# patrickltobing/shallow-wavenet

Measured on AMD Instinct MI355X. Metric: decoded samples/sec (22.05 kHz Laplacian AR decode, whole job), higher is better.
Workload: dtype f32

## Files before the change

shallow_wavenet_amd/csrc/swn_decode_bl6w.hip:

```cpp
#include <type_traits>
#include "swn_decode_bl6_common.hpp"
#include "swn_decode_internal.hpp"

namespace {

using namespace swn_bl6;

constexpr int NG = 256;
constexpr int S = 128;
constexpr int O1 = 128;

template <int LPC_, bool EXT_>
struct Tw {
    static constexpr int LPC = LPC_;
    static constexpr bool EXT = EXT_;
    using Ext = Tw<LPC_, true>;
    static constexpr int NO = 2 + LPC_;
    static constexpr int WN = cmax(1, LPC_) + 1;
    static constexpr int ring_len(int l) { return pow2ceil((1 << l) + 1); }
    static constexpr int ring_off(int l) { int o = 0; for (int i = 0; i < l; ++i) o += ring_len(i) * H; return o; }
    static constexpr int PF = L * 2 * H;
    static constexpr int NZC = 64, NZB = 4;
    static constexpr int o_ring = 0;
    static constexpr int o_hcat = o_ring + ring_off(L);
    static constexpr int o_gp = o_hcat + L * H;
    static constexpr int o_bx = o_gp + 2 * PF;
    static constexpr int o_bd = o_bx + L * 2 * H;
    static constexpr int o_old = o_bd + L * 2 * H;
    static constexpr int o_wup = o_old + 2 * L * 2 * H;
    static constexpr int o_skip = o_wup + 256;
    static constexpr int o_p2 = o_skip + S;
    static constexpr int o_tnz = o_p2 + 4 * NO;
    static constexpr int o_cz = o_tnz + r4(NZB * NZC);
    static constexpr int o_w2 = o_cz + 5 * H;
    static constexpr int o_bias = o_w2 + NO * S + r4(NO);
    static constexpr int o_w1 = o_bias + S + O1;
    static constexpr int o_wl = o_w1 + 8 * O1 * 16;
    static constexpr int o_h0w = o_wl + 8 * NG * 4;
    static constexpr int o_end = o_h0w + 3 * H;
    static constexpr size_t lds_bytes = (size_t)o_end * sizeof(float);
    static constexpr int sess_old = ring_off(L);
    static constexpr int sess_win = sess_old + 2 * L * 2 * H;
    static constexpr int sess_floats = sess_win + r4(WN);
};

__device__ __forceinline__ float sum_quads(float v) {
    v += dpp_f<0x124>(v);
    v += dpp_f<0x128>(v);
    float w = v;
    asm("s_nop 1\n\tv_permlane16_swap_b32 %0, %1" : "+v"(v), "+v"(w));
    v += w;
    w = v;
    asm("s_nop 1\n\tv_permlane32_swap_b32 %0, %1" : "+v"(v), "+v"(w));
    return v + w;
}
template <class T, int LAYER>
__device__ __forceinline__ void layer_a(float* lds, const float (&w)[2][16], const int q, const float wj, const int pb, const int ta,
                                        const float* xr) {
    const int o = ta >> 2, p = ta & 3, pr = p & 1;
    const float e_old = lds[T::o_old + (q & 1) * (L * 2 * H) + LAYER * 2 * H + pr * H + o];
    const float e_gx = fmaf(wj, lds[T::o_gp + pb + LAYER * 2 * H + pr * H + o], lds[T::o_bx + LAYER * 2 * H + pr * H + o]);
    const float e_hp = xr[o];
    float az = 0.f, ac = 0.f;
#pragma unroll
    for (int m = 0; m < 4; ++m) {
        const float4 x = *reinterpret_cast<const float4*>(xr + 16 * p + 4 * m);
        az = fmaf(w[0][4 * m], x.x, az); ac = fmaf(w[1][4 * m], x.x, ac);
        az = fmaf(w[0][4 * m + 1], x.y, az); ac = fmaf(w[1][4 * m + 1], x.y, ac);
        az = fmaf(w[0][4 * m + 2], x.z, az); ac = fmaf(w[1][4 * m + 2], x.z, ac);
        az = fmaf(w[0][4 * m + 3], x.w, az); ac = fmaf(w[1][4 * m + 3], x.w, ac);
    }
    az = sum4(az); ac = sum4(ac);
    __builtin_amdgcn_sched_barrier(0);
    if (p < 2) {
        const float sa = (p == 0 ? az : ac) + e_old;
        const float v = e_gx * sa;
        float res;
        if (fabsf(v) > 9.02f && p == 1) {
            res = copysignf(1.f, v);
        } else {
            const float e = exp_c(p == 0 ? -v : -2.f * fabsf(v));
            const float r = rcp_c(1.f + e);
            res = p == 0 ? r : copysignf((1.f - e) * r, v);
        }
        const float c = dpp_f<0xF5>(res);
        if (p == 0) {
            const float hn = (1.f - res) * c + res * e_hp;
            if (LAYER + 1 < L) {
                constexpr int R2 = T::ring_len(LAYER + 1 < L ? LAYER + 1 : LAYER);
                lds[T::o_ring + T::ring_off(LAYER + 1 < L ? LAYER + 1 : LAYER) + (q & (R2 - 1)) * H + o] = hn;
            }
            lds[T::o_hcat + LAYER * H + o] = hn;
        }
    }
    __builtin_amdgcn_sched_barrier(0);
}

template <class T, int LAYER, int MB = 4>
__device__ __forceinline__ void older_sum(const float* lds, const float (&w)[2][16], const int qn, const int tb, float& az, float& ac) {
    constexpr int dil = 1 << LAYER;
    constexpr int R = T::ring_len(LAYER);
    const int p = tb & 3;
    const float* ring = lds + T::o_ring + T::ring_off(LAYER);
    az = 0.f; ac = 0.f;
#pragma unroll
    for (int m = 0; m < 4; ++m) {
        const float4 x = *reinterpret_cast<const float4*>(ring + ((qn - dil) & (R - 1)) * H + 16 * p + 4 * m);
        float4 w0, w1;
        if (LAYER < L - 1) {
            w0 = make_float4(w[0][4 * m], w[0][4 * m + 1], w[0][4 * m + 2], w[0][4 * m + 3]);
            w1 = make_float4(w[1][4 * m], w[1][4 * m + 1], w[1][4 * m + 2], w[1][4 * m + 3]);
        } else {
            w0 = *reinterpret_cast<const float4*>(lds + T::o_wl + (m * NG + tb) * 4);
            w1 = *reinterpret_cast<const float4*>(lds + T::o_wl + ((4 + m) * NG + tb) * 4);
        }
        az = fmaf(w0.x, x.x, az); ac = fmaf(w1.x, x.x, ac);
        az = fmaf(w0.y, x.y, az); ac = fmaf(w1.y, x.y, ac);
        az = fmaf(w0.z, x.z, az); ac = fmaf(w1.z, x.z, ac);
        az = fmaf(w0.w, x.w, az); ac = fmaf(w1.w, x.w, ac);
        if (MB < 4 && m % MB == MB - 1) __builtin_amdgcn_sched_barrier(0);
    }
    az = sum4(az); ac = sum4(ac);
}
template <class T, int LAYER>
__device__ __forceinline__ void older_store(float* lds, const int qn, const int tb, const float az, const float ac) {
    const int o = tb >> 2, p = tb & 3, pr = p & 1;
    lds[T::o_old + (qn & 1) * (L * 2 * H) + LAYER * 2 * H + pr * H + o] = (p == 0 ? az : ac) + lds[T::o_bd + LAYER * 2 * H + pr * H + o];
}
template <class T, int LAYER, int MB = 4>
__device__ __forceinline__ void older_b(float* lds, const float (&w)[2][16], const int qn, const int tb) {
    float az, ac;
    older_sum<T, LAYER, MB>(lds, w, qn, tb, az, ac);
    if ((tb & 3) < 2) older_store<T, LAYER>(lds, qn, tb, az, ac);
}
template <int... LS> struct Layers {};
template <class T, int NW, int... LS>
__device__ __forceinline__ void older_bn(Layers<LS...>, float* lds, const float (&w)[NW][2][16], const int qn, const int tb) {
    static_assert(((LS < NW) && ...), "register-resident halves only");
    float az[sizeof...(LS)], ac[sizeof...(LS)];
    int k = 0;
    ((older_sum<T, LS>(lds, w[LS], qn, tb, az[k], ac[k]), ++k), ...);
    if ((tb & 3) < 2) {
        k = 0;
        ((older_store<T, LS>(lds, qn, tb, az[k], ac[k]), ++k), ...);
    }
}

template <class T, int LAYER>
__device__ __forceinline__ void older_rows(const float* lds, const int qn, const int tb, float4 (&x)[4]) {
    constexpr int dil = 1 << LAYER;
    constexpr int R = T::ring_len(LAYER);
    const float* row = lds + T::o_ring + T::ring_off(LAYER) + ((qn - dil) & (R - 1)) * H + 16 * (tb & 3);
#pragma unroll
    for (int m = 0; m < 4; ++m) x[m] = *reinterpret_cast<const float4*>(row + 4 * m);
}
__device__ __forceinline__ void older_sum_x(const float (&w)[2][16], const float4 (&x)[4], float& az, float& ac) {
    az = 0.f; ac = 0.f;
#pragma unroll
    for (int m = 0; m < 4; ++m) {
        az = fmaf(w[0][4 * m], x[m].x, az); ac = fmaf(w[1][4 * m], x[m].x, ac);
        az = fmaf(w[0][4 * m + 1], x[m].y, az); ac = fmaf(w[1][4 * m + 1], x[m].y, ac);
        az = fmaf(w[0][4 * m + 2], x[m].z, az); ac = fmaf(w[1][4 * m + 2], x[m].z, ac);
        az = fmaf(w[0][4 * m + 3], x[m].w, az); ac = fmaf(w[1][4 * m + 3], x[m].w, ac);
    }
    az = sum4(az); ac = sum4(ac);
}
template <class T, int... LS>
__device__ __forceinline__ void older_rows_n(Layers<LS...>, const float* lds, const int qn, const int tb, float4 (&x)[sizeof...(LS)][4]) {
    int k = 0;
    ((older_rows<T, LS>(lds, qn, tb, x[k]), ++k), ...);
}
template <class T, int NW, int... LS>
__device__ __forceinline__ void older_bn_x(Layers<LS...>, float* lds, const float (&w)[NW][2][16], const float4 (&x)[sizeof...(LS)][4],
                                           const int qn, const int tb) {
    static_assert(((LS < NW) && ...), "register-resident halves only");
    float az[sizeof...(LS)], ac[sizeof...(LS)];
    int k = 0;
    ((older_sum_x(w[LS], x[k], az[k], ac[k]), ++k), ...);
    if ((tb & 3) < 2) {
        k = 0;
        ((older_store<T, LS>(lds, qn, tb, az[k], ac[k]), ++k), ...);
    }
}

template <int LAYER>
__device__ __forceinline__ void skip_issue_b(__amdgpu_buffer_rsrc_t wsk2, float4 (&wsl)[8], const int tb, const unsigned step0) {
    const int r = tb >> 2, hp = tb & 3;
#pragma unroll
    for (int ps = 0; ps < 2; ++ps)
#pragma unroll
        for (int mm = 0; mm < 4; ++mm)
            wsl[ps * 4 + mm] = buf_ld4(wsk2, (unsigned)((r + 64 * ps) * 4 + hp) * 16u, (unsigned)((LAYER * 4 + mm) * S) * 64u + step0);
}
template <class T, int LAYER>
__device__ __forceinline__ void skip_roll_b(const float* lds, __amdgpu_buffer_rsrc_t wsk2, float4 (&wsl)[8], float (&sacc)[2], const int tb,
                                            const unsigned step0) {
    static_assert(LAYER >= 1 && LAYER < L, "slice LAYER - 1 in flight, slice LAYER to request");
    const int r = tb >> 2, hp = tb & 3;
#pragma unroll
    for (int hf = 0; hf < 2; ++hf) {
#pragma unroll
        for (int mm = 2 * hf; mm < 2 * hf + 2; ++mm) {
            const float4 x = *reinterpret_cast<const float4*>(lds + T::o_hcat + (LAYER - 1) * H + 16 * mm + 4 * hp);
#pragma unroll
            for (int ps = 0; ps < 2; ++ps) {
                const float4 w = wsl[ps * 4 + mm];
                sacc[ps] = fmaf(w.x, x.x, sacc[ps]); sacc[ps] = fmaf(w.y, x.y, sacc[ps]);
                sacc[ps] = fmaf(w.z, x.z, sacc[ps]); sacc[ps] = fmaf(w.w, x.w, sacc[ps]);
            }
        }
        __builtin_amdgcn_sched_barrier(0);
#pragma unroll
        for (int mm = 2 * hf; mm < 2 * hf + 2; ++mm)
#pragma unroll
            for (int ps = 0; ps < 2; ++ps)
                wsl[ps * 4 + mm] = buf_ld4(wsk2, (unsigned)((r + 64 * ps) * 4 + hp) * 16u, (unsigned)((LAYER * 4 + mm) * S) * 64u + step0);
        __builtin_amdgcn_sched_barrier(0);
    }
    asm volatile("" : "+v"(sacc[0]), "+v"(sacc[1]));
}
template <class T>
__device__ __forceinline__ void skip_last_b(float* lds, const float4 (&wsl)[8], const float (&sacc)[2], const int tb) {
    const int r = tb >> 2, hp = tb & 3;
    float part[2][4];
#pragma unroll
    for (int mm = 0; mm < 4; ++mm) {
        const float4 x = *reinterpret_cast<const float4*>(lds + T::o_hcat + (L - 1) * H + 16 * mm + 4 * hp);
#pragma unroll
        for (int ps = 0; ps < 2; ++ps) {
            const float4 w = wsl[ps * 4 + mm];
            part[ps][mm] = fmaf(w.w, x.w, fmaf(w.z, x.z, fmaf(w.y, x.y, w.x * x.x)));
        }
    }
    float s[2];
#pragma unroll
    for (int ps = 0; ps < 2; ++ps) s[ps] = sacc[ps] + ((part[ps][0] + part[ps][1]) + (part[ps][2] + part[ps][3]));
    const float t0 = s[0] + dpp_f<0xB1>(s[0]), t1 = s[1] + dpp_f<0xB1>(s[1]);
    const float v = (hp < 2 ? t0 : t1) + dpp_f<0x4E>(hp < 2 ? t1 : t0);
    if ((hp & 1) == 0) lds[T::o_skip + r + 32 * hp] = fmaxf(v, 0.f);
}

using OlderMerged = Layers<3, 4>;
using OlderOut1 = Layers<0, 1, 2>;

template <class T, bool GA, bool STREAM, bool POOL = false>
__device__ __forceinline__ void decode_body(const Bl6Args& a, float* lds) {
    constexpr bool EXT = T::EXT;
    static_assert(!STREAM || EXT, "streamed chunks run the extended mode");
    constexpr bool grpA = GA;
    const int tid = threadIdx.x, b = POOL ? 0 : blockIdx.x;
    __builtin_assume(GA ? tid < NG : tid >= NG);
    const int tg = tid & (NG - 1);
    const float* __restrict__ P = a.P;
    const int U = a.U;
    const int s0 = STREAM ? a.step0 : 0;
    const bool resume = STREAM && a.resume;
    const int fb0 = STREAM ? s0 / U : 0;

    for (int e = tid; e < T::o_end; e += NT) lds[e] = 0.f;
    __syncthreads();
    for (int e = tid; e < L * 2 * H; e += NT) {
        lds[T::o_bx + e] = P[a.y.bx + e];
        const float bd = P[a.y.bd + e];
        lds[T::o_bd + e] = bd;
        lds[T::o_old + e] = bd;
    }
    for (int e = tid; e < U; e += NT) lds[T::o_wup + e] = P[a.y.wup + e];
    for (int e = tid; e < H; e += NT) lds[T::o_cz + e] = P[a.y.cb + e];
    for (int e = tid; e < S; e += NT) lds[T::o_bias + e] = P[a.y.bsk + e];
    for (int e = tid; e < O1; e += NT) lds[T::o_bias + S + e] = P[a.y.b1 + e];
    for (int e = tid; e < 2 * H; e += NT) { lds[T::o_cz + H + e] = P[a.y.cv + e]; lds[T::o_cz + 3 * H + e] = P[a.y.cc + e]; }
    for (int e = tid; e < T::NO * S; e += NT) lds[T::o_w2 + e] = P[a.y.w2 + (size_t)(e / S) * r4(S) + (e % S)];
    for (int e = tid; e < T::NO; e += NT) lds[T::o_w2 + T::NO * S + e] = P[a.y.b2 + e];
    for (int e = tid; e < 8 * O1 * 16; e += NT) lds[T::o_w1 + e] = P[a.y.w12 + e];
    const __amdgpu_buffer_rsrc_t condr =
        make_rsrc(a.cond + (size_t)b * a.Tf * a.N, (unsigned)((size_t)a.Tf * a.N * sizeof(float)));
    auto load_frame = [&](int fr) {
        float* dst = lds + T::o_gp + (fr & 1) * T::PF;
#pragma unroll
        for (int it = 0; it < (T::PF / 4 + NT - 1) / NT; ++it) {
            const int e4 = it * NT + tid;
            if (e4 < T::PF / 4)
                *reinterpret_cast<float4*>(dst + 4 * e4) =
                    buf_ld4(condr, (unsigned)tid * 16u, (unsigned)(fr * a.N * 4 + it * NT * 16));
        }
    };
    for (int fr = fb0; fr < fb0 + 2 && fr < a.Tf; ++fr) load_frame(fr);
    constexpr int NWR = grpA ? L : L - 1;
    float wreg[NWR][2][16];
    {
        const int o = tg >> 2, p = tg & 3, k = grpA ? 1 : 0;
#pragma unroll
        for (int l = 0; l < L; ++l)
#pragma unroll
            for (int r = 0; r < 2; ++r) {
                const float4* src = reinterpret_cast<const float4*>(P + a.y.wd + (((size_t)l * 2 * H + o + r * H) * 2 + k) * H + 16 * p);
#pragma unroll
                for (int v = 0; v < 4; ++v) {
                    const float4 t = src[v];
                    if (l == L - 1 && !grpA) {
                        *reinterpret_cast<float4*>(lds + T::o_wl + ((r * 4 + v) * NG + tg) * 4) = t;
                    } else {
                        float (&wr)[16] = wreg[l < NWR ? l : 0][r];
                        wr[4 * v] = t.x; wr[4 * v + 1] = t.y; wr[4 * v + 2] = t.z; wr[4 * v + 3] = t.w;
                    }
                }
            }
    }
    __syncthreads();
    const float* sess_b = STREAM ? a.sess + (size_t)b * T::sess_floats : nullptr;
    int tcp = tid;
    asm volatile("" : "+v"(tcp));
    if (resume) {
        for (int e = tcp; e < T::ring_off(L); e += NT) lds[T::o_ring + e] = sess_b[e];
        for (int e = tcp; e < 2 * L * 2 * H; e += NT) lds[T::o_old + e] = sess_b[T::sess_old + e];
        __syncthreads();
    }

    int fb = fb0, tb0 = fb0 * U;
    const int n_pro = RF;
    auto cond_taps = [&](int q, float& wj, int& pb) {
        const int t0 = q - RF;
        const int tlo = t0 < 0 ? 0 : t0;
        if (tlo >= tb0 + U) {
            fb += 1; tb0 += U;
            if (fb + 1 < a.Tf) load_frame(fb + 1);
        }
        int rel = tlo - tb0;
        int fsel = fb;
        if (rel >= U) { rel -= U; fsel = fb + 1; }
        rel = rel < U ? rel : U - 1;
        wj = lds[T::o_wup + rel];
        pb = (fsel & 1) * T::PF;
    };

    auto input_seed = [&](int q) {
        if (tid < H) {
            const int o = tid;
            float acc = c_b;
#pragma unroll
            for (int k = 0; k < 2; ++k) {
                const int r = q - (1 - k);
                if (r >= 0) acc += fmaf(k ? c_v1 : c_v0, 0.f, k ? c_c1 : c_c0);
            }
            lds[T::o_ring + (q & 1) * H + o] = ssign(acc);
        }
    };
    float win[T::WN];
#pragma unroll
    for (int k = 0; k < T::WN; ++k) win[k] = 0.f;
    if (EXT && a.seed) win[T::WN - 1] = reinterpret_cast<const float*>(a.seed)[b];
    if (resume) {
#pragma unroll
        for (int k = 0; k < T::WN; ++k) win[k] = sess_b[T::sess_win + k];
    }
    const int wv = __builtin_amdgcn_readfirstlane(tg >> 6);
    float kcb = 0.f, kv0 = 0.f, kv1 = 0.f, kc0 = 0.f, kc1 = 0.f;
    if (grpA) { const int o = tg & (H - 1); kcb = c_b; kv0 = c_v0; kv1 = c_v1; kc0 = c_c0; kc1 = c_c1; }
    auto h0_row = [&](int qn) -> float* {
        return wv == 0 ? lds + T::o_ring + (qn & 1) * H : lds + T::o_h0w + (wv - 1) * H;
    };
    auto input_gen = [&](int qn) {
        if constexpr (grpA) {
            float acc = kcb;
            acc += fmaf(kv0, win[T::WN - 2], kc0);
            acc += fmaf(kv1, win[T::WN - 1], kc1);
            h0_row(qn)[tg & (H - 1)] = ssign(acc);
            asm volatile("s_waitcnt lgkmcnt(0)" ::: "memory");
        }
    };
    float e_next = 0.f;
    auto noise_load = [&](int c) {
        const int step = c * T::NZC + tid - 64;
        if (step < a.n_steps) e_next = a.noise[(size_t)b * a.n_steps + step];
    };
    auto noise_chunk = [&](int c) {
        if (grpA && tid >= 64 && tid < 128) {
            const int k = tid - 64, step = c * T::NZC + k;
            if (step < a.n_steps) {
                const float e = EXT ? swn_noise_laplace_at(a.nz, b, step, s0 + step, 0, a.n_steps, 1) : e_next;
                const float sg = (e > 0.f) ? 1.f : ((e < 0.f) ? -1.f : 0.f);
                lds[T::o_tnz + (c & (T::NZB - 1)) * T::NZC + k] = sg * log1pf(-2.f * fabsf(e));
            }
            if (!EXT) noise_load(c + 1);
        }
    };
    if (!EXT && grpA && tid >= 64 && tid < 128) noise_load(0);
    noise_chunk(0);
    noise_chunk(1);

    const __amdgpu_buffer_rsrc_t wsk2 = make_rsrc(P + a.y.wsk2, (unsigned)(L * S * 64 * sizeof(float)));

#ifdef SWN_STAMP
    unsigned long long tw[9] = {0, 0, 0, 0, 0, 0, 0, 0, 0}, tv[6] = {0, 0, 0, 0, 0, 0}, tstep = 0, tlast = 0, tbeg = 0;
#define SWN_BAR(k) { tw[k] += __builtin_amdgcn_s_memtime() - tlast; lds_barrier(); tlast = __builtin_amdgcn_s_memtime(); }
#define SWN_WAIT_STAMP(k) { asm volatile("" :: "v"(wsl[0].x)); tv[k] += __builtin_amdgcn_s_memtime() - tlast; }
#define SWN_PRE(k) { tw[k] += __builtin_amdgcn_s_memtime() - tlast; asm volatile("s_waitcnt lgkmcnt(0)" ::: "memory"); }
#define SWN_BAR_KEEP(k, N) { lds_barrier_keep<N>(); tlast = __builtin_amdgcn_s_memtime(); }
#else
#define SWN_BAR(k) lds_barrier();
#define SWN_WAIT_STAMP(k)
#define SWN_PRE(k)
#define SWN_BAR_KEEP(k, N) lds_barrier_keep<N>();
#endif
#define SWN_PHASE(LAYER, GEN, X0)                                                                                     \
    if constexpr (grpA) layer_a<T, LAYER>(lds, wreg[LAYER], q, wj, pb, tg,                                             \
                                          LAYER == 0 ? (X0) : lds + T::o_ring + T::ring_off(LAYER) +                   \
                                                                  (q & (T::ring_len(LAYER) - 1)) * H);                 \
    else {                                                                                                             \
        if (GEN) {    \
                      \
                      \
            if (LAYER == 0) skip_issue_b<0>(wsk2, wsl, tg, step0);                                                     \
            else { SWN_WAIT_STAMP(LAYER > 0 ? LAYER - 1 : 0) skip_roll_b<T, (LAYER > 0 ? LAYER : 1)>(lds, wsk2, wsl, sacc, tg, step0); } \
            __builtin_amdgcn_sched_barrier(0);                                                                         \
        }                                                                                                              \
        if (!(GEN)) older_b<T, LAYER>(lds, wreg[LAYER < NWR ? LAYER : 0], q + 1, tg);                                  \
        else if (LAYER == 0) older_bn<T>(OlderMerged{}, lds, wreg, q + 1, tg);                                         \
        __builtin_amdgcn_sched_barrier(0);                                                                             \
    }                                                                                                                  \
    if (GEN) { SWN_BAR(LAYER) } else lds_barrier();

#pragma unroll 1
    for (int q = resume ? n_pro : 0; q < n_pro; ++q) {
        float wj; int pb;
        float4 wsl[8]; float sacc[2]; const unsigned step0 = 0;
        cond_taps(q, wj, pb);
        input_seed(q);
        lds_barrier();
        const float* x0 = lds + T::o_ring + (q & 1) * H;
        SWN_PHASE(0, false, x0) SWN_PHASE(1, false, x0) SWN_PHASE(2, false, x0) SWN_PHASE(3, false, x0)
        SWN_PHASE(4, false, x0) SWN_PHASE(5, false, x0)
        (void)wsl; (void)sacc; (void)step0;
    }

    input_gen(RF + s0);
#ifdef SWN_STAMP
    tlast = tbeg = __builtin_amdgcn_s_memtime();
#endif
    auto gen_step = [&](const int i) __attribute__((always_inline)) {
        const int q = RF + s0 + i;
        float wj; int pb;
        cond_taps(q, wj, pb);
        float4 wsl[8];
        float sacc[2] = {0.f, 0.f};
        if constexpr (!grpA) {
            const float bs0 = lds[T::o_bias + (tg >> 2)], bs1 = lds[T::o_bias + (tg >> 2) + 64];
            if ((tg & 3) == 0) { sacc[0] = bs0; sacc[1] = bs1; }
        }
        unsigned step0 = 0;
        asm volatile("" : "+s"(step0));
        const float* x0 = h0_row(q);
        SWN_PHASE(0, true, x0) SWN_PHASE(1, true, x0) SWN_PHASE(2, true, x0) SWN_PHASE(3, true, x0)
        SWN_PHASE(4, true, x0) SWN_PHASE(5, true, x0)
        constexpr bool ROLL1 = T::LPC == 0;
        float4 xo[3][4];
        float4 w1e[2][2];
        if constexpr (!grpA) {
            SWN_WAIT_STAMP(5) skip_last_b<T>(lds, wsl, sacc, tg);
            SWN_PRE(6)
            lds_fence_compiler();
            __builtin_amdgcn_sched_barrier(0);
            older_rows_n<T>(OlderOut1{}, lds, q + 1, tg, xo);
            __builtin_amdgcn_sched_barrier(0);
            SWN_BAR_KEEP(6, 12)
        } else {
            older_b<T, L - 1, 2>(lds, wreg[L - 1], q + 1, tg + (int)step0);
            if constexpr (ROLL1) {
                SWN_PRE(6)
                lds_fence_compiler();
                __builtin_amdgcn_sched_barrier(0);
#pragma unroll
                for (int mm = 0; mm < 2; ++mm)
#pragma unroll
                    for (int r = 0; r < 2; ++r)
                        w1e[mm][r] = *reinterpret_cast<const float4*>(lds + T::o_w1 + ((mm * O1 + (tg >> 2) + 64 * r) * 4 + (tg & 3)) * 4);
                __builtin_amdgcn_sched_barrier(0);
                SWN_BAR_KEEP(6, 4)
            } else {
                SWN_BAR(6)
            }
        }
        if constexpr (grpA) {
            const int hr = tg >> 2, hp = tg & 3;
            float a0 = 0.f, a1 = 0.f, b0 = 0.f, b1 = 0.f;
            auto X = [&](int mm) { return *reinterpret_cast<const float4*>(lds + T::o_skip + 16 * mm + 4 * hp); };
            auto W = [&](int mm, int r) { return *reinterpret_cast<const float4*>(lds + T::o_w1 + ((mm * O1 + hr + 64 * r) * 4 + hp) * 4); };
            auto fma8 = [&](int mm, const float4& x0, const float4& w0, const float4& w1) {
                float& acc = (mm & 1) ? a1 : a0;
                float& bcc = (mm & 1) ? b1 : b0;
                acc = fmaf(w0.x, x0.x, acc); acc = fmaf(w0.y, x0.y, acc); acc = fmaf(w0.z, x0.z, acc); acc = fmaf(w0.w, x0.w, acc);
                bcc = fmaf(w1.x, x0.x, bcc); bcc = fmaf(w1.y, x0.y, bcc); bcc = fmaf(w1.z, x0.z, bcc); bcc = fmaf(w1.w, x0.w, bcc);
            };
            if constexpr (ROLL1) {
                float4 xr[3] = {X(0), X(1), X(2)};
                __builtin_amdgcn_sched_barrier(0);
#pragma unroll
                for (int mm = 0; mm < 8; ++mm) {
                    fma8(mm, xr[mm % 3], w1e[mm % 2][0], w1e[mm % 2][1]);
                    __builtin_amdgcn_sched_barrier(0);
                    if (mm + 2 < 8) { w1e[mm % 2][0] = W(mm + 2, 0); w1e[mm % 2][1] = W(mm + 2, 1); }
                    if (mm + 3 < 8) xr[mm % 3] = X(mm + 3);
                    __builtin_amdgcn_sched_barrier(0);
                }
            } else {
#pragma unroll
                for (int mm = 0; mm < 8; ++mm) {
                    fma8(mm, X(mm), W(mm, 0), W(mm, 1));
                    if ((mm & 3) == 3) __builtin_amdgcn_sched_barrier(0);
                }
            }
            const float v = sum4(a0 + a1), u = sum4(b0 + b1);
            const float o1a = fmaxf(v + lds[T::o_bias + S + hr], 0.f), o1b = fmaxf(u + lds[T::o_bias + S + hr + 64], 0.f);
#pragma unroll
            for (int j = 0; j < (T::NO + 3) / 4; ++j) {
                const int k = hp + 4 * j, kc = k < T::NO ? k : T::NO - 1;
                const float* w2 = lds + T::o_w2 + kc * S;
                const float b2 = lds[T::o_w2 + T::NO * S + kc];
                const float pz = sum_quads(fmaf(w2[hr + 64], o1b, fmaf(w2[hr], o1a, tg < 4 ? b2 : 0.f)));
                if ((tg & 63) < 4 && k < T::NO) lds[T::o_p2 + 4 * k + wv] = pz;
            }
        } else {
            older_bn_x<T>(OlderOut1{}, lds, wreg, xo, q + 1, tg);
        }
        SWN_BAR(7)
        if constexpr (grpA) {
            const int ln = tg & 63;
            float tz = 0.f;
            if constexpr (!EXT) tz = lds[T::o_tnz + (i & (T::NZB * T::NZC - 1))];
            float fv = 0.f;
            if (a.forced) fv = reinterpret_cast<const float*>(a.forced)[(size_t)b * a.n_steps + i];
            const float4 pz = *reinterpret_cast<const float4*>(lds + T::o_p2 + 4 * (ln < T::NO ? ln : T::NO - 1));
            const float acc = (pz.x + pz.y) + (pz.z + pz.w);
            float o2[T::NO];
#pragma unroll
            for (int k = 0; k < T::NO; ++k) o2[k] = __builtin_bit_cast(float, __builtin_amdgcn_readlane(__builtin_bit_cast(int, acc), k));
            {
#pragma clang fp contract(off)
                float* outp = reinterpret_cast<float*>(a.out) + (size_t)b * a.n_steps + (size_t)i;
                const float mu = o2[0];
                const float bsc = sigm(o2[1]);
                float lpv = 0.f;
#pragma unroll
                for (int k = 0; k < T::LPC; ++k) lpv += o2[2 + T::LPC - 1 - k] * win[T::WN - T::LPC + k];
                const float t = bsc * (EXT ? lds[T::o_tnz + ((i >> 6) & (T::NZB - 1)) * T::NZC + (i & (T::NZC - 1))] : tz);
                float sv = (T::LPC > 0) ? (lpv + mu) - t : mu - t;
                sv = fminf(fmaxf(sv, -1.f), 1.f);
                float fd = a.forced ? fv : sv;
                asm volatile("" : "+v"(fd));
#pragma unroll
                for (int k = 0; k + 1 < T::WN; ++k) win[k] = win[k + 1];
                win[T::WN - 1] = fd;
                if (tid == 0) outp[0] = sv;
            }
            if (HEADS_ON && a.heads && wv == 0 && ln < T::NO) a.heads[((size_t)b * a.n_steps + i) * T::NO + ln] = acc;
        }
        if (i + 1 < a.n_steps) input_gen(q + 1);
#ifdef SWN_STAMP
        if constexpr (grpA) tw[8] += __builtin_amdgcn_s_memtime() - tlast;
#endif
    };
#pragma unroll 1
    for (int i0 = 0; i0 < a.n_steps; i0 += T::NZC) {
        noise_chunk((i0 >> 6) + 2);
        const int iend = i0 + T::NZC < a.n_steps ? i0 + T::NZC : a.n_steps;
#pragma unroll 1
        for (int i = i0; i < iend; ++i) gen_step(i);
    }
#ifdef SWN_STAMP
    { const unsigned long long tn = __builtin_amdgcn_s_memtime(); tw[0] += tn - tlast; tstep = tn - tbeg; }
#endif
    if constexpr (STREAM) {
        __syncthreads();
        float* so = a.sess + (size_t)b * T::sess_floats;
        tcp = tid;
        asm volatile("" : "+v"(tcp));
        for (int e = tcp; e < T::ring_off(L); e += NT) so[e] = lds[T::o_ring + e];
        for (int e = tcp; e < 2 * L * 2 * H; e += NT) so[T::sess_old + e] = lds[T::o_old + e];
        if (tid == 0) {
#pragma unroll
            for (int k = 0; k < T::WN; ++k) so[T::sess_win + k] = win[k];
        }
    }
#undef SWN_PHASE
#undef SWN_BAR
#undef SWN_WAIT_STAMP
#undef SWN_PRE
#undef SWN_BAR_KEEP
#ifdef SWN_STAMP
    if ((tid == 0 || tid == 64 || tid == NG) && b == 0 && a.heads) {
        float* h = a.heads + (tid == 0 ? 0 : tid == 64 ? 30 : 10);
        for (int k = 0; k < 9; ++k) h[k] = (float)((double)tw[k] / (double)a.n_steps);
        if (tid == 0) h[9] = (float)((double)tstep / (double)a.n_steps);
        else if (tid == NG) for (int k = 0; k < 6; ++k) h[10 + k] = (float)((double)tv[k] / (double)a.n_steps);
    }
#endif
}

template <class T, bool STREAM = false>
__global__ __launch_bounds__(NT) void decode_bl6w_kernel(const Bl6Args a) {
    extern __shared__ __attribute__((aligned(16))) float lds[];
    if (threadIdx.x < NG) decode_body<T, true, STREAM>(a, lds);
    else decode_body<T, false, STREAM>(a, lds);
}

template <class T, bool MODELS = false>
__global__ __launch_bounds__(NT) void decode_bl6w_pool_kernel(
    const typename std::conditional<MODELS, Bl6PoolModelsArgs, Bl6PoolArgs>::type p) {
    extern __shared__ __attribute__((aligned(16))) float lds[];
    static_assert(T::EXT, "pools run the extended mode");
    Bl6Args a = p.c;
    if constexpr (MODELS) a.P = swn_pool_model(p.m);
    if (!swn_pool_entry_args(a, p.t, 1, 1, T::NO)) return;
    a.sess += (size_t)swn_pool_slot(p.t) * T::sess_floats;
    if (threadIdx.x < NG) decode_body<T, true, true, true>(a, lds);
    else decode_body<T, false, true, true>(a, lds);
}

bool bl6w_applies(const SwnGeom& g) {
    return g.bl6 && g.U <= 256 && g.U >= 2 && !g.audio_in && g.kind == SWN_KIND_LAPLACE && g.S == 128 && g.O1 == 128 &&
           g.seg == 1 && (g.lpc == 0 || g.lpc == 4);
}

template <class F>
int with_tw(const SwnGeom& g, F&& f) {
    if (!bl6w_applies(g)) return SWN_E_UNSUPPORTED;
    if (g.lpc == 0) return f(Tw<0, false>{});
    return f(Tw<4, false>{});
}

}

int swn_decode_bl6w_run(const SwnDecodeCall& c) {
    const hipStream_t st = c.hip_stream;
    if (c.pool) {
        Bl6PoolModelsArgs p;
        fill_args(p.c, c);
        p.t = *c.pool;
        if (c.models) p.m = *c.models;
        return with_tw(c.g, [&](auto tw) {
            using T = typename decltype(tw)::Ext;
            if (c.models)
                return launch_kernel(decode_bl6w_pool_kernel<T, true>, T::lds_bytes, c.batch, p, st, "swn_decode_pool_chunk_models(bl6w)");
            const Bl6PoolArgs& p1 = p;
            return launch_kernel(decode_bl6w_pool_kernel<T>, T::lds_bytes, c.batch, p1, st, "swn_decode_pool_chunk(bl6w)");
        });
    }
    Bl6Args a;
    fill_args(a, c);
    return with_tw(c.g, [&](auto t) {
        using T = decltype(t);
        using X = typename T::Ext;
        static_assert(T::lds_bytes <= 160 * 1024 && X::lds_bytes <= 160 * 1024, "LDS budget");
        if (c.stream) return launch_kernel(decode_bl6w_kernel<X, true>, X::lds_bytes, a.B, a, st, "swn_decode(bl6w)");
        if (wants_ext(a)) return launch_kernel(decode_bl6w_kernel<X>, X::lds_bytes, a.B, a, st, "swn_decode(bl6w)");
        return launch_kernel(decode_bl6w_kernel<T>, T::lds_bytes, a.B, a, st, "swn_decode(bl6w)");
    });
}

size_t swn_decode_bl6w_session_floats(const SwnGeom& g) {
    int n = 0;
    with_tw(g, [&](auto t) { n = decltype(t)::sess_floats; return SWN_OK; });
    return (size_t)n;
}
```

Before: 373,800.

## Precompute next-step conditioning taps and prefetch out_2 weights in decode loop

```diff
diff --git a/shallow_wavenet_amd/csrc/swn_decode_bl6w.hip b/shallow_wavenet_amd/csrc/swn_decode_bl6w.hip
--- a/shallow_wavenet_amd/csrc/swn_decode_bl6w.hip
+++ b/shallow_wavenet_amd/csrc/swn_decode_bl6w.hip
@@ -55,10 +55,10 @@
     return v + w;
 }
 template <class T, int LAYER>
-__device__ __forceinline__ void layer_a(float* lds, const float (&w)[2][16], const int q, const float wj, const int pb, const int ta,
-                                        const float* xr) {
+__device__ __forceinline__ void layer_a(float* lds, const float (&w)[2][16], const int q, const float wj, const int pb, const int po,
+                                        const int ta, const float* xr) {
     const int o = ta >> 2, p = ta & 3, pr = p & 1;
-    const float e_old = lds[T::o_old + (q & 1) * (L * 2 * H) + LAYER * 2 * H + pr * H + o];
+    const float e_old = lds[T::o_old + po + LAYER * 2 * H + pr * H + o];
     const float e_gx = fmaf(wj, lds[T::o_gp + pb + LAYER * 2 * H + pr * H + o], lds[T::o_bx + LAYER * 2 * H + pr * H + o]);
     const float e_hp = xr[o];
     float az = 0.f, ac = 0.f;
@@ -357,16 +357,16 @@
     const int wv = __builtin_amdgcn_readfirstlane(tg >> 6);
     float kcb = 0.f, kv0 = 0.f, kv1 = 0.f, kc0 = 0.f, kc1 = 0.f;
     if (grpA) { const int o = tg & (H - 1); kcb = c_b; kv0 = c_v0; kv1 = c_v1; kc0 = c_c0; kc1 = c_c1; }
-    auto h0_row = [&](int qn) -> float* {
-        return wv == 0 ? lds + T::o_ring + (qn & 1) * H : lds + T::o_h0w + (wv - 1) * H;
-    };
-    auto input_gen = [&](int qn) {
+    auto h0_row = [&](int qn) -> int {
+        return wv == 0 ? T::o_ring + (qn & 1) * H : T::o_h0w + (wv - 1) * H;
+    };
+    auto input_gen = [&](int row) {
         if constexpr (grpA) {
             float acc = kcb;
             acc += fmaf(kv0, win[T::WN - 2], kc0);
             acc += fmaf(kv1, win[T::WN - 1], kc1);
-            h0_row(qn)[tg & (H - 1)] = ssign(acc);
-            asm volatile("s_waitcnt lgkmcnt(0)" ::: "memory");
+            lds[row + (tg & (H - 1))] = ssign(acc);
+            lds_fence_compiler();
         }
     };
     float e_next = 0.f;
@@ -404,7 +404,7 @@
 #define SWN_BAR_KEEP(k, N) lds_barrier_keep<N>();
 #endif
 #define SWN_PHASE(LAYER, GEN, X0)                                                                                     \
-    if constexpr (grpA) layer_a<T, LAYER>(lds, wreg[LAYER], q, wj, pb, tg,                                             \
+    if constexpr (grpA) layer_a<T, LAYER>(lds, wreg[LAYER], q, wj, pb, po, tg,                                         \
                                           LAYER == 0 ? (X0) : lds + T::o_ring + T::ring_off(LAYER) +                   \
                                                                   (q & (T::ring_len(LAYER) - 1)) * H);                 \
     else {                                                                                                             \
@@ -426,6 +426,7 @@
         float wj; int pb;
         float4 wsl[8]; float sacc[2]; const unsigned step0 = 0;
         cond_taps(q, wj, pb);
+        const int po = (q & 1) * (L * 2 * H);
         input_seed(q);
         lds_barrier();
         const float* x0 = lds + T::o_ring + (q & 1) * H;
@@ -434,14 +435,35 @@
         (void)wsl; (void)sacc; (void)step0;
     }
 
-    input_gen(RF + s0);
+    int rel_c = s0 - fb0 * U;
+    bool fill_c = false;
+    float wj_c = 0.f;
+    int pb_c = 0, po_c = 0, x0_c = 0;
+    auto taps_ahead = [&](int qn) {
+        wj_c = lds[T::o_wup + rel_c];
+        pb_c = (fb & 1) * T::PF;
+        po_c = (qn & 1) * (L * 2 * H);
+        x0_c = h0_row(qn);
+        asm volatile("" : "+s"(pb_c), "+s"(po_c), "+s"(x0_c));
+    };
+    auto frame_advance = [&]() {
+        rel_c += 1;
+        const bool cross = rel_c >= U;
+        if (cross) { rel_c = 0; fb += 1; }
+        fill_c = cross && fb + 1 < a.Tf;
+    };
+    if constexpr (grpA) taps_ahead(RF + s0);
+    input_gen(x0_c);
 #ifdef SWN_STAMP
     tlast = tbeg = __builtin_amdgcn_s_memtime();
 #endif
     auto gen_step = [&](const int i) __attribute__((always_inline)) {
         const int q = RF + s0 + i;
-        float wj; int pb;
-        cond_taps(q, wj, pb);
+        const float wj = wj_c;
+        const int pb = pb_c, po = po_c;
+        if constexpr (grpA) {
+            if (fill_c) load_frame(fb + 1);
+        }
         float4 wsl[8];
         float sacc[2] = {0.f, 0.f};
         if constexpr (!grpA) {
@@ -450,7 +472,7 @@
         }
         unsigned step0 = 0;
         asm volatile("" : "+s"(step0));
-        const float* x0 = h0_row(q);
+        const float* x0 = lds + x0_c;
         SWN_PHASE(0, true, x0) SWN_PHASE(1, true, x0) SWN_PHASE(2, true, x0) SWN_PHASE(3, true, x0)
         SWN_PHASE(4, true, x0) SWN_PHASE(5, true, x0)
         constexpr bool ROLL1 = T::LPC == 0;
@@ -492,7 +514,10 @@
                 acc = fmaf(w0.x, x0.x, acc); acc = fmaf(w0.y, x0.y, acc); acc = fmaf(w0.z, x0.z, acc); acc = fmaf(w0.w, x0.w, acc);
                 bcc = fmaf(w1.x, x0.x, bcc); bcc = fmaf(w1.y, x0.y, bcc); bcc = fmaf(w1.z, x0.z, bcc); bcc = fmaf(w1.w, x0.w, bcc);
             };
+            float e_b1[2] = {0.f, 0.f}, e_w2[2] = {0.f, 0.f}, e_b2 = 0.f;
+            const int e_kc = hp < T::NO ? hp : T::NO - 1;
             if constexpr (ROLL1) {
+                static_assert(T::NO <= 4, "one round of out_2 rows");
                 float4 xr[3] = {X(0), X(1), X(2)};
                 __builtin_amdgcn_sched_barrier(0);
 #pragma unroll
@@ -501,6 +526,11 @@
                     __builtin_amdgcn_sched_barrier(0);
                     if (mm + 2 < 8) { w1e[mm % 2][0] = W(mm + 2, 0); w1e[mm % 2][1] = W(mm + 2, 1); }
                     if (mm + 3 < 8) xr[mm % 3] = X(mm + 3);
+                    if (mm == 5) {
+                        e_b1[0] = lds[T::o_bias + S + hr]; e_b1[1] = lds[T::o_bias + S + hr + 64];
+                        e_w2[0] = lds[T::o_w2 + e_kc * S + hr]; e_w2[1] = lds[T::o_w2 + e_kc * S + hr + 64];
+                    }
+                    if (mm == 6) e_b2 = lds[T::o_w2 + T::NO * S + e_kc];
                     __builtin_amdgcn_sched_barrier(0);
                 }
             } else {
@@ -511,14 +541,20 @@
                 }
             }
             const float v = sum4(a0 + a1), u = sum4(b0 + b1);
-            const float o1a = fmaxf(v + lds[T::o_bias + S + hr], 0.f), o1b = fmaxf(u + lds[T::o_bias + S + hr + 64], 0.f);
-#pragma unroll
-            for (int j = 0; j < (T::NO + 3) / 4; ++j) {
-                const int k = hp + 4 * j, kc = k < T::NO ? k : T::NO - 1;
-                const float* w2 = lds + T::o_w2 + kc * S;
-                const float b2 = lds[T::o_w2 + T::NO * S + kc];
-                const float pz = sum_quads(fmaf(w2[hr + 64], o1b, fmaf(w2[hr], o1a, tg < 4 ? b2 : 0.f)));
-                if ((tg & 63) < 4 && k < T::NO) lds[T::o_p2 + 4 * k + wv] = pz;
+            if constexpr (ROLL1) {
+                const float o1a = fmaxf(v + e_b1[0], 0.f), o1b = fmaxf(u + e_b1[1], 0.f);
+                const float pz = sum_quads(fmaf(e_w2[1], o1b, fmaf(e_w2[0], o1a, tg < 4 ? e_b2 : 0.f)));
+                if ((tg & 63) < 4 && hp < T::NO) lds[T::o_p2 + 4 * hp + wv] = pz;
+            } else {
+                const float o1a = fmaxf(v + lds[T::o_bias + S + hr], 0.f), o1b = fmaxf(u + lds[T::o_bias + S + hr + 64], 0.f);
+#pragma unroll
+                for (int j = 0; j < (T::NO + 3) / 4; ++j) {
+                    const int k = hp + 4 * j, kc = k < T::NO ? k : T::NO - 1;
+                    const float* w2 = lds + T::o_w2 + kc * S;
+                    const float b2 = lds[T::o_w2 + T::NO * S + kc];
+                    const float pz = sum_quads(fmaf(w2[hr + 64], o1b, fmaf(w2[hr], o1a, tg < 4 ? b2 : 0.f)));
+                    if ((tg & 63) < 4 && k < T::NO) lds[T::o_p2 + 4 * k + wv] = pz;
+                }
             }
         } else {
             older_bn_x<T>(OlderOut1{}, lds, wreg, xo, q + 1, tg);
@@ -531,31 +567,36 @@
             float fv = 0.f;
             if (a.forced) fv = reinterpret_cast<const float*>(a.forced)[(size_t)b * a.n_steps + i];
             const float4 pz = *reinterpret_cast<const float4*>(lds + T::o_p2 + 4 * (ln < T::NO ? ln : T::NO - 1));
+            __builtin_amdgcn_sched_barrier(0);
+            frame_advance();
+            taps_ahead(q + 1);
+            __builtin_amdgcn_sched_barrier(0);
             const float acc = (pz.x + pz.y) + (pz.z + pz.w);
             float o2[T::NO];
 #pragma unroll
             for (int k = 0; k < T::NO; ++k) o2[k] = __builtin_bit_cast(float, __builtin_amdgcn_readlane(__builtin_bit_cast(int, acc), k));
+            float sv;
             {
 #pragma clang fp contract(off)
-                float* outp = reinterpret_cast<float*>(a.out) + (size_t)b * a.n_steps + (size_t)i;
                 const float mu = o2[0];
                 const float bsc = sigm(o2[1]);
                 float lpv = 0.f;
 #pragma unroll
                 for (int k = 0; k < T::LPC; ++k) lpv += o2[2 + T::LPC - 1 - k] * win[T::WN - T::LPC + k];
                 const float t = bsc * (EXT ? lds[T::o_tnz + ((i >> 6) & (T::NZB - 1)) * T::NZC + (i & (T::NZC - 1))] : tz);
-                float sv = (T::LPC > 0) ? (lpv + mu) - t : mu - t;
+                sv = (T::LPC > 0) ? (lpv + mu) - t : mu - t;
                 sv = fminf(fmaxf(sv, -1.f), 1.f);
                 float fd = a.forced ? fv : sv;
                 asm volatile("" : "+v"(fd));
 #pragma unroll
                 for (int k = 0; k + 1 < T::WN; ++k) win[k] = win[k + 1];
                 win[T::WN - 1] = fd;
-                if (tid == 0) outp[0] = sv;
-            }
+            }
+            if (i + 1 < a.n_steps) input_gen(x0_c);
+            __builtin_amdgcn_sched_barrier(0);
+            if (tid == 0) reinterpret_cast<float*>(a.out)[(size_t)b * a.n_steps + (size_t)i] = sv;
             if (HEADS_ON && a.heads && wv == 0 && ln < T::NO) a.heads[((size_t)b * a.n_steps + i) * T::NO + ln] = acc;
         }
-        if (i + 1 < a.n_steps) input_gen(q + 1);
 #ifdef SWN_STAMP
         if constexpr (grpA) tw[8] += __builtin_amdgcn_s_memtime() - tlast;
 #endif
```

Result: faster. 378,900 (median of 6 runs) (+1.4%).
